# lis-epfl/multi_agent_pkgs

Measured on AMD Instinct MI355X. Metric: agent QP-replans/sec, higher is better.
Workload: dtype f64

## Files before the change

### __graft_entry__.py

```python
import os
import subprocess
import sys

ROOT = os.path.dirname(os.path.abspath(__file__))
if ROOT not in sys.path:
    sys.path.insert(0, ROOT)


def build() -> None:
    csrc = os.path.join(ROOT, "multi_agent_pkgs_amd", "csrc")
    subprocess.check_call(["make", "-C", csrc, "-s"])
    subprocess.check_call(["make", "-C", os.path.join(ROOT, "oracle"), "-s"])
    subprocess.check_call(["make", "-C", os.path.join(ROOT, "tests", "wave_emu"), "-s"])
    subprocess.check_call(["make", "-C", os.path.join(ROOT, "examples"), "-s"])
    subprocess.check_call(["make", "-C", os.path.join(ROOT, "ros"), "-s"])
    subprocess.check_call(["make", "-C", os.path.join(ROOT, "tests", "ros_shim"), "-s"])
    import multi_agent_pkgs_amd
    from multi_agent_pkgs_amd import lib
    L = lib.load()
    for name in lib.EXPORTS:
        getattr(L, name)
    print("build ok: libhdsm.so version 0x%x" % L.hdsm_version())


def smoke() -> None:
    import numpy as np
    sys.path.insert(0, os.path.join(ROOT, "tests"))
    import problems
    from multi_agent_pkgs_amd import lib
    from multi_agent_pkgs_amd.params import agile_params
    from oracle import pyoracle as orc

    prm = agile_params(10, max_rows_static=18)
    sn = problems.swarm_snapshot(prm, 16, seed=7, turn=True)
    args = [sn[k] for k in ("agent_id", "state", "ref", "n_poly", "n_rows", "A", "b", "plans", "has_plan")]
    sol = lib.Solver(prm, 16, 16, device=0)
    g = sol.replan(*args)
    o = orc.replan(prm, *args)
    assert (g["status"] == o["status"]).all(), (g["status"], o["status"])
    ok = o["status"] != 2
    dt = float(np.abs(g["traj"] - o["traj"])[ok].max())
    dj = float(np.abs(g["obj"] - o["obj"])[ok].max())
    assert dt < 1e-6 and dj < 1e-6, (dt, dj)
    print("smoke ok: 16 agent-replans on cuda:0, max |traj - oracle| = %.2e, |obj - oracle| = %.2e" % (dt, dj))


# ... 5 lines not shown
```

### multi_agent_pkgs_amd/csrc/hdsm_consts.cpp

```cpp
#include "hdsm_consts.h"

#include <cmath>
#include <cstdlib>
#include <cstring>
#include <vector>

namespace hdsm {
namespace {

struct M3 {
  double m[3][3];
};
M3 eye() {
  M3 r{};
  for (int i = 0; i < 3; ++i) r.m[i][i] = 1;
  return r;
}
M3 mul(const M3& a, const M3& b) {
  M3 r{};
  for (int i = 0; i < 3; ++i)
    for (int j = 0; j < 3; ++j)
      for (int k = 0; k < 3; ++k) r.m[i][j] += a.m[i][k] * b.m[k][j];
  return r;
}
// ... 38 lines not shown
      char* end = nullptr;
      const long v = std::strtol(e, &end, 10);
      if (end != e && *end == 0 && v >= lo && v <= hi) *out = (int32_t)v;
    }
  };
  auto env_real = [](const char* name, double lo, double hi, double* out) {
    if (const char* e = std::getenv(name)) {
      char* end = nullptr;
      const double v = std::strtod(e, &end);
      if (end != e && *end == 0 && v >= lo && v <= hi) *out = v;
    }
  };
  if (prm->presweep < 0 || prm->presweep > 2) return fail(err, "presweep must be 0 (automatic), 1 (never) or 2 (always)");
  if (prm->branch_rule < 0 || prm->branch_rule > 1) return fail(err, "branch_rule must be 0 (most infeasible) or 1 (first in time)");
  if (prm->stage_radius < 0 || prm->time_limit_s < 0) return fail(err, "stage_radius / time_limit_s must not be negative");
  if (!(prm->mip_gap >= 0) || prm->mip_gap >= 1) return fail(err, "mip_gap must be in [0, 1)");
  c->cand_tau = prm->stage_radius > 0 ? prm->stage_radius : 0.6;
  env_real("HDSM_CAND_TAU", 0.01, 10.0, &c->cand_tau);
  c->branch_rule = prm->branch_rule == 0 ? 1 : 0;
  env_int("HDSM_BRANCH_RULE", 0, 1, &c->branch_rule);
  c->presweep = prm->presweep == 0 ? 2 : (prm->presweep == 1 ? 0 : 1);
  env_int("HDSM_PRESWEEP", 0, 2, &c->presweep);
  c->hot_tau = 1e30;
  env_real("HDSM_HOT_TAU", 1e-3, 1e30, &c->hot_tau);
  c->pick_rule = 1;
  env_int("HDSM_PICK_RULE", 0, 1, &c->pick_rule);
  c->box_cut = 1;
  env_int("HDSM_BOX_CUT", 0, 1, &c->box_cut);
  c->scanner = 1;
  env_int("HDSM_SCANNER", 0, 2, &c->scanner);
  c->child_bound = 1, c->overlap_sweep = 1;
  env_int("HDSM_OVERLAP_SWEEP", 0, 1, &c->overlap_sweep);
  env_int("HDSM_CHILD_BOUND", 0, 1, &c->child_bound);
  c->dominance = 1;
  env_int("HDSM_DOMINANCE", 0, 1, &c->dominance);
  c->mip_gap = prm->mip_gap;
  c->leaf_mfma = 1;
  env_int("HDSM_LEAF_MFMA", 0, 1, &c->leaf_mfma);
  c->time_ticks = 0;
  c->r_u = prm->r_u;
  for (int k = 0; k < 6; ++k) c->wx[k] = prm->r_x[k], c->wn[k] = prm->r_n[k];
  for (int ax = 0; ax < 3; ++ax) {
    c->lbu[ax] = prm->u_lb[ax], c->ubu[ax] = prm->u_ub[ax];
    for (int comp = 1; comp < 3; ++comp) {
      c->lbs[comp][ax] = prm->x_lb[3 * comp + ax];
      c->ubs[comp][ax] = prm->x_ub[3 * comp + ax];
    }
  }
  c->radius = prm->drone_radius;
  const double kk = prm->drone_radius / prm->drone_z_offset;
  c->k2m1 = kk * kk - 1.0;
  c->pert = prm->plane_perturb;

  for (int ax = 0; ax < 3; ++ax) {
    M3 Ac{};
    Ac.m[0][1] = 1, Ac.m[1][1] = -prm->drag[ax], Ac.m[1][2] = 1;
    const double dt = prm->dt;
    M3 Ad, Bm;
    if (!prm->rk4) {
      Ad = axpy(eye(), dt, Ac);
      Bm = eye();
      for (auto& row : Bm.m)
        for (double& v : row) v *= dt;
    } else {
      const M3 A1 = Ac, A2 = mul(Ac, Ac), A3 = mul(A2, Ac), A4 = mul(A3, Ac);
      Ad = axpy(axpy(axpy(axpy(eye(), dt, A1), dt * dt / 2, A2), dt * dt * dt / 6, A3), dt * dt * dt * dt / 24, A4);
// ... 227 lines not shown
```

### multi_agent_pkgs_amd/csrc/hdsm_core.h

```cpp
#pragma once
#include <math.h>
#include <stdint.h>

#include <hip/hip_runtime.h>
#define HD __device__ __forceinline__
#define HDN __device__ __noinline__
#define PAR_FOR(i, cnt) for (int i = tid_here(); i < (cnt); i += (int)blockDim.x)
#define HDSM_UNROLL _Pragma("unroll")
#define SYNC() __syncthreads()
#define IS_T0 (HDSM_TX == 0)
namespace hdsm {
__device__ __forceinline__ int atomic_inc_i32(int* p) { return atomicAdd(p, 1); }
__device__ __forceinline__ unsigned tx() {
  unsigned t = threadIdx.x;
#if defined(__HIP_DEVICE_COMPILE__)
  asm volatile("" : "+v"(t));
#endif
  return t;
}
}
#define HDSM_TX (hdsm::tx())
#if defined(__HIP_DEVICE_COMPILE__)
#define HDSM_KERNARG_WORD __attribute__((address_space(4))) long long
#else
#define HDSM_KERNARG_WORD long long
#endif

#include "hdsm_types.h"

namespace hdsm {

enum { GI_OK = 0, GI_INFEASIBLE = 1, GI_CUTOFF = 2, GI_ITERLIM = 3, GI_DONE = 4, GI_TIMELIM = 5 };
constexpr int NODE_CHUNK = 4;
constexpr int TREE_MARK = 32;
constexpr int WARM_CERT = 1 << 30;
enum { FLAG_NODE_LIMIT = 1, FLAG_ITER_LIMIT = 2, FLAG_TIME_LIMIT = 4, FLAG_STAGING_OVERFLOW = 8 };
enum { ST_OPTIMAL = 0, ST_LIMIT = 1, ST_NO_SOLUTION = 2, ST_PENDING = 3 };

enum { K_U = 0, K_S = 1, K_P = 2, K_C = 3, K_E = 4 };
HD int mk_id(int kind, int payload) { return (kind << 28) | payload; }
HD int id_kind(int id) { return (id >> 28) & 7; }
HD int id_payload(int id) { return id & 0x0fffffff; }
HD int mk_kc(int slot, int m) { return mk_id(K_C, (m << 12) | slot); }
HD int kc_slot(int payload) { return payload & 0xfff; }
HD int kc_m(int payload) { return payload >> 12; }

constexpr int LISTCAP = 768;

struct alignas(8) MW {
  int32_t m;
  float w;
};
static_assert(sizeof(MW) == 8, "hand-over records copy MW as one 8-byte word");
HD MW mk_mw(const double (*kap)[4], double nx, double ny, double nz, int m) {
  const double q = nx * nx * kap[m][0] + ny * ny * kap[m][1] + nz * nz * kap[m][2];
  return MW{m, q > 1e-60 ? (float)(1.0 / sqrt(q)) : 1e30f};
}

template <int NV, int CMAX, bool SMALL = false>
struct Shm {
  static_assert(CMAX <= 4096, "the slot of a staged row must fit the 12 bits kc_slot() reads");
  static constexpr int PM = SMALL ? 4 : MAXP, RSM = SMALL ? 20 : MAXRS, LC = SMALL ? 512 : LISTCAP;
  static constexpr int LDT = (NV <= 32) ? 34 : NV + 2;
  alignas(16) double T[2];
  alignas(16) double U[NV * LDT];
  alignas(16) double dvec[NV + 2];
  alignas(16) double dvz[NV + 2];
  double gz[3][3][2 * MAXH];
  double x0[NV];
  double fx0;
  int32_t cand_src[CMAX];
  int32_t inc_act[NV], inc_nact;
  int32_t st_sph, st_pairs;
  long long t_start;
#ifdef HDSM_PROFILE
  long long prof_acc[24];
  long long prof_last;
  long long prof_last1;
#endif
  double x[NV], lam[NV], w[NV], grad[NV];
  double inc_x[NV];
  double g[3][3][MAXH];
  double fr[3][MAXH + 1][3];
  double ref[MAXH][6];
  double st[MAXH + 1][9];
  double cprev[MAXH][3];
  alignas(16) double sp[PM][RSM][4];
  double keys[MAXH][PM];
  static constexpr int HTS = NV / 3;
  double br_lb[HTS][PM], br_pv[HTS][PM];
  int32_t br_pk[HTS][PM];
  HD double& lb_at(int item) { return red_v[item]; }
  HD double& pv_at(int item) { return red_v[64 + item]; }
  HD int32_t& pk_at(int item) { return reinterpret_cast<int32_t*>(&red_v[128])[item]; }
  static_assert(128 + 32 <= MAXT, "the leaf test's per-(step, polyhedron) values fit the reduction scratch");
// ... 2 lines not shown
  double first_v;
  double lb_top1, lb_top2;
  int32_t lb_step;
  alignas(16) double cand[CMAX][4];
  double red_v[MAXT];
  double br_f[MAXH];
  double state0[9];
  double f, inc_f, f0;
  MW cand_mw[CMAX];
  int32_t act[NV];
  int32_t sp_rows[PM];
  int32_t assign[MAXH], contain[MAXH], inc_assign[MAXH];
  int32_t br_step[MAXH], br_pos[MAXH], br_cnt[MAXH], br_order[MAXH][PM];
  int32_t q, neq_done, ncand, n_poly, level, have_inc, fixed_bad, overflow;
  int32_t inf_id;
  unsigned long long nogood[NOGOODS];
  int32_t n_nogood, ng_skipped, ng_global;
  int32_t lb_skipped;
  int32_t ncold;
  double f_box;
  double inc_shared;
  int32_t wanted_raw;
  int32_t nviol;
  int32_t warm_head;
  int32_t warm_ncand;
  int32_t leaf_pick;
  int32_t sp_dom, dom_done;
  int32_t forced;
  double* snap;
  int32_t node_res;
  int32_t rc, iters_sh;
  int32_t cmd;
  int32_t nlist;
  int32_t grp[2];
  int32_t list[LC];
  double sw[5];
  double sw_ref[MAXH + 1][3];
  double sw_tau;
  double sw_d2;
  double bnd[24];
  static_assert(MAXT >= 16 + KCOLS + 8, "the reduction scratch doubles as the set-up's input vector");
  HD double* vin() { return &red_v[16]; }
  double part_v[4];
  double part_key[4];
  double part_tol;
  int32_t part_id[4];
  int32_t part_norm;
  double kap[MAXH + 1][4];
  Args args;
};

HD bool tasc_plane_eval(const Consts& c, const double* cp, const double* op, double* out) {
  const double dx = op[0] - cp[0], dy = op[1] - cp[1], dz = op[2] - cp[2];
  const double n2 = dx * dx + dy * dy + dz * dz;
  if (!(n2 > 0)) return false;
  const double nrm = sqrt(n2), inv = 1.0 / nrm;
  const double hx = dx * inv, hy = dy * inv, hz = dz * inv;
  const double sd = c.radius / sqrt(1.0 + c.k2m1 * hz * hz);
  const double back = 0.5 * fmin(2.0 * sd, nrm);
  const double qx = 0.5 * (cp[0] + op[0]) - back * hx;
  const double qy = 0.5 * (cp[1] + op[1]) - back * hy;
  const double qz = 0.5 * (cp[2] + op[2]) - back * hz;
  const double fx = hx + c.pert * (hy - hz) - c.pert * hz;
  const double fy = hy - c.pert * hx;
  const double fz = hz + c.pert * hx + c.pert * hx;
  out[0] = fx, out[1] = fy, out[2] = fz;
// ... 738 lines not shown
        s.f0 = t0;
        s.fx0 = t0 + 0.5 * t1;
        s.f = s.fx0 + 0.5 * t2;
        s.inc_nact = 0;
      }
    }
    SYNC();
    SU_PROF(15)

#ifdef HDSM_PROFILE
    const long long t_setup_ = clock64() - t_begin_;
#endif
#ifdef HDSM_TIMELINE
    const long long tl_setup_ = (long long)wall_clock64();
    long long tl_warm_ = 0, tl_sweep_ = 0, tl_run_ = 0, tl_leaf_ = 0;
    int tl_warm_it_ = 0, tl_runs_ = 0;
#define TL_T0 const long long tl_t0_ = (long long)wall_clock64();
#define TL_ADD(acc) acc += (long long)wall_clock64() - tl_t0_;
#else
#define TL_T0
#define TL_ADD(acc)
#endif
    int iters = 0, nodes = 1, sweeps = 0;
    bool warm_cert = false;
    if (a.warm != nullptr && np > 0) warm_cert = (s.warm_head & WARM_CERT) != 0;
#if defined(HDSM_PROFILE)
    long long t_warm_ = 0;
    int it_warm_ = 0;
#endif
    bool limit = false, handed_over = false;
    int rec_slot = -1;
    unsigned flags = 0;
    bool run = np > 0;
    if (IS_T0) s.sw_tau = 0.0;
    bool item_run = false;
    if (item >= 0) {
      const SplitRec& rc = a.recs[item >> 8];
      const int L = (item >> 3) & 15, pos = item & 7;
      const int nh = rc.ncand, ncl = rc.ncold;
      const int64_t rbase = (int64_t)(item >> 8) * a.rows_cap;
      SYNC();
      PAR_FOR(k, nh + ncl) {
        const int slot = k < nh ? k : CMAX - ncl + (k - nh);
        const double* src = a.rec_cand + (rbase + k) * 4;
        s.cand[slot][0] = src[0], s.cand[slot][1] = src[1], s.cand[slot][2] = src[2], s.cand[slot][3] = src[3];
        *reinterpret_cast<long long*>(&s.cand_mw[slot]) = a.rec_mw[rbase + k];
        s.cand_src[slot] = a.rec_src[rbase + k];
      }
      PAR_FOR(k, 3 * (N + 1)) s.sw_ref[k / 3][k % 3] = rc.sw_ref[k / 3][k % 3];
      PAR_FOR(k, rc.n_nogood) s.nogood[k] = rc.nogood[k];
      PAR_FOR(l, L + 1) {
        s.br_step[l] = rc.br_step[l], s.br_cnt[l] = 0, s.br_pos[l] = 0, s.br_f[l] = rc.br_f[l];
        s.assign[rc.br_step[l]] = l < L ? rc.assign[rc.br_step[l]] : rc.br_order[L][pos];
      }
      if (IS_T0) {
        s.ncand = nh, s.ncold = ncl, s.n_nogood = rc.n_nogood, s.sw_tau = rc.sw_tau, s.level = L + 1;
        s.sp_dom = rc.sp_dom, s.dom_done = 1;
        const int code = rc.br_pk[L][pos];
        s.first_id = code >= 0 ? mk_id(K_P, (rc.br_step[L] << 7) | code) : -1, s.first_v = rc.br_pv[L][pos];
        const unsigned long long bits = __hip_atomic_load(&a.inc_bits[inst], __ATOMIC_RELAXED, __HIP_MEMORY_SCOPE_AGENT);
        s.inc_shared = __longlong_as_double((long long)bits);
      }
      SYNC();
      item_run = run && nh + ncl <= CMAX && !(rc.br_lb[L][pos] >= cutoff(s, c));
      if (item_run) snapshot_io(s, c, R, const_cast<double*>(rc.snap) + (int64_t)L * SNAP_STRIDE, false);
      if (IS_T0) s.neq_done = 6;
      run = item_run;
// ... 537 lines not shown
```

### multi_agent_pkgs_amd/csrc/hdsm_types.h

```cpp
#pragma once
#include <stdint.h>

namespace hdsm {

constexpr int MAXH = 16;
constexpr int MAXP = 8;
constexpr int MAXRS = 32;
constexpr int MAXNV = 3 * MAXH;
constexpr int MAXT = 256;
constexpr int KCOLS = 9 + 6 * MAXH;
constexpr int KROWS = 3 * MAXNV + 12;
constexpr int SPLIT_N_MAX = 30;
constexpr int KCH = 3 + 2 * MAXH;
constexpr double ABSENT = 1e20;
constexpr double DINF = 1e300;

struct Consts {
  int32_t N, n, P, RS;
  int32_t max_nodes, max_iters;
  int32_t presweep;
  int32_t leaf_mfma;
  int32_t branch_rule;
  int32_t pick_rule;
  int32_t box_cut;
  int32_t scanner;
  int32_t child_bound;
  int32_t overlap_sweep;
  double tol, ftol_fixed, cand_tau, hot_tau;
  double mip_gap;
  long long time_ticks;
  double r_u, wx[6], wn[6];
  double lbu[3], ubu[3];
  double lbs[3][3], ubs[3][3];
  double radius, k2m1, pert;
  double Ad[3][3][3], Bd[3][3];
  double g[3][3][MAXH];
  int32_t pinned_steps;
  int32_t dominance;
  double phi[3][MAXH + 1][3][3];
  double Hinv[MAXNV * MAXNV];
  double J0[MAXNV * MAXNV];
  double Jeq[MAXNV * MAXNV];
  double Req[36], Ueq[36];
  double Meq[MAXNV * 6];
  double Seq[36];
  double KT[KCOLS * KROWS];
  double KTC[KCH * KROWS];
  int32_t kax[KROWS];
  double JeqP[MAXNV * 64];
  double hrow1[MAXNV];
  double wu[MAXNV];
  double ws[3][3][MAXH + 1];
  double kap[MAXH + 1][4];
};

constexpr int NOGOODS = 48;
constexpr int ITEMS_PER_REC = 64;

struct SplitRec {
  int32_t inst, level, ncand, ncold, n_nogood, first_item, n_items, nodes_done, sweeps_done, truncated;
// ... 77 lines not shown
```

### multi_agent_pkgs_amd/csrc/hdsm_wave_gi.h

```cpp
#pragma once
#include <hip/hip_runtime.h>

#include "hdsm_types.h"

namespace hdsm {

template <int CTRL>
__device__ __forceinline__ double dpp64(double v) {
  int lo = __double2loint(v), hi = __double2hiint(v);
  lo = __builtin_amdgcn_mov_dpp(lo, CTRL, 0xf, 0xf, true);
  hi = __builtin_amdgcn_mov_dpp(hi, CTRL, 0xf, 0xf, true);
  return __hiloint2double(hi, lo);
}
__device__ __forceinline__ double bcast64(double v, int lane) {
  const int lo = __builtin_amdgcn_readlane(__double2loint(v), lane);
  const int hi = __builtin_amdgcn_readlane(__double2hiint(v), lane);
  return __hiloint2double(hi, lo);
}
__device__ __forceinline__ double wave_max64(double v) {
  v = fmax(v, dpp64<0x121>(v));
  v = fmax(v, dpp64<0x122>(v));
  v = fmax(v, dpp64<0x124>(v));
  v = fmax(v, dpp64<0x128>(v));
  return fmax(fmax(bcast64(v, 0), bcast64(v, 16)), fmax(bcast64(v, 32), bcast64(v, 48)));
// ... 68 lines not shown
  if (hot) {
    slot = __hip_atomic_fetch_add(&ncand, 1, __ATOMIC_ACQ_REL, __HIP_MEMORY_SCOPE_WORKGROUP);
    const int other = __hip_atomic_load(&ncold, __ATOMIC_RELAXED, __HIP_MEMORY_SCOPE_WORKGROUP);
    return slot >= 0 && slot < CMAX - other;
  }
  slot = CMAX - 1 - __hip_atomic_fetch_add(&ncold, 1, __ATOMIC_ACQ_REL, __HIP_MEMORY_SCOPE_WORKGROUP);
  const int other = __hip_atomic_load(&ncand, __ATOMIC_RELAXED, __HIP_MEMORY_SCOPE_WORKGROUP);
  return slot < CMAX && slot >= other && slot >= 0;
#else
  slot = hot ? atomicAdd(&ncand, 1) : CMAX - 1 - atomicAdd(&ncold, 1);
  const bool fits = (hot ? slot < CMAX - __hip_atomic_load(&ncold, __ATOMIC_RELAXED, __HIP_MEMORY_SCOPE_WORKGROUP)
                         : slot >= __hip_atomic_load(&ncand, __ATOMIC_RELAXED, __HIP_MEMORY_SCOPE_WORKGROUP)) &&
                    slot >= 0 && slot < CMAX;
  HDSM_STAGE_AUDIT_CLAIM(slot, fits);
  return fits;
#endif
}

__device__ __forceinline__ void keep_in_loop(int& v) {
#if defined(__HIP_DEVICE_COMPILE__)
  asm volatile("" : "+v"(v));
#else
  (void)v;
#endif
}

__device__ __forceinline__ int tid_here() {
  int t = (int)HDSM_TX;
  keep_in_loop(t);
  return t;
}

__device__ __forceinline__ void keep_here(double& v) {
#if defined(__HIP_DEVICE_COMPILE__)
  asm volatile("" : "+v"(v));
#else
  (void)v;
#endif
}

template <class T>
__device__ __forceinline__ T* keep_in_loop(T* p) {
#if defined(__HIP_DEVICE_COMPILE__)
  asm volatile("" : "+v"(p));
#endif
  return p;
}

struct alignas(16) D2 {
  double x, y;
};

#if defined(__HIP_DEVICE_COMPILE__)
template <class T>
using GPtr = __attribute__((address_space(1))) T*;
template <class T>
__device__ __forceinline__ GPtr<const T> gptr(const T* p) { return (GPtr<const T>)p; }
template <class T>
__device__ __forceinline__ GPtr<T> gptr(T* p) { return (GPtr<T>)p; }
#else
template <class T>
using GPtr = T*;
template <class T>
__device__ __host__ inline GPtr<const T> gptr(const T* p) { return p; }
template <class T>
__device__ __host__ inline GPtr<T> gptr(T* p) { return p; }
// ... 87 lines not shown
        w.has = g.has_plan[k], w.ox = op[0], w.oy = op[1], w.oz = op[2];
      }
    }
  }

  struct LaneReq {
    double hrow;
    double wu, sb_w[2];
    int comp[2], axs[2], ii[2];
  };
  static __device__ __forceinline__ LaneReq init_lane_request(const Consts& c, int lane) {
    const int n = c.n;
    LaneReq q;
    q.wu = c.wu[lane < n ? lane : 0];
    q.hrow = c.hrow1[lane < n ? lane : 0];
#pragma unroll
    for (int e = 0; e < 2; ++e) {
      const int idx = lane + 64 * e, k = idx % 6;
      q.ii[e] = idx / 6 + 1, q.comp[e] = 1 + k / 3, q.axs[e] = k % 3;
      q.sb_w[e] = c.ws[q.axs[e]][q.comp[e]][q.ii[e] <= MAXH ? q.ii[e] : 0];
    }
    return q;
  }
  static __device__ __forceinline__ void init_lane(Regs& R, const Consts& c, int lane, const LaneReq& q) {
    const int N = c.N;
    const int n_sb = 6 * (N - 1);
    R.ax = row_of(lane) / N, R.kk = row_of(lane) % N;
    R.wu = (float)q.wu;
#pragma unroll
    for (int e = 0; e < 2; ++e) {
      const bool on = lane + 64 * e < n_sb;
      R.sb_id[e] = on ? ((q.ii[e] << 5) | (q.comp[e] << 3) | (q.axs[e] << 1)) : -1;
      R.sb_w[e] = (float)q.sb_w[e];
    }
  }

  template <int PART = 0>
  static __device__ __forceinline__ void states(S& s, const Regs& R, int lane, int N) {
    if constexpr (SPLIT) {
      constexpr bool P0 = PART != 2, VA = PART != 1;
      const int row = lane & 31, h = lane >> 5;
      const bool on = row < 3 * N;
      const int ax = on ? R.ax : 0, m = on ? R.kk + 1 : 1;
      double acc0 = 0, acc1 = 0, acc2 = 0;
      if (h == 0) {
        if constexpr (P0) acc0 = s.fr[ax][m][0];
        if constexpr (VA) acc1 = s.fr[ax][m][1], acc2 = s.fr[ax][m][2];
      }
      const double* xx = s.x + ax * N;
      const double* g0 = &s.gz[ax][0][MAXH + m - 1];
      const double* g1 = &s.gz[ax][1][MAXH + m - 1];
      const double* g2 = &s.gz[ax][2][MAXH + m - 1];
      constexpr int HH = HT / 2;
      static_assert(HT % 2 == 0, "the split kernel halves the horizon capacity");
#pragma unroll
      for (int k = 0; k < HH; ++k) {
        const int kk = h * HH + k;
        const double xk = xx[kk];
        if constexpr (P0) acc0 += g0[-kk] * xk;
        if constexpr (VA) acc1 += g1[-kk] * xk, acc2 += g2[-kk] * xk;
      }
      if constexpr (P0) acc0 = half_sum64(acc0);
      if constexpr (VA) acc1 = half_sum64(acc1), acc2 = half_sum64(acc2);
      if (on && h == 0) {
        if constexpr (P0) s.st[m][ax] = acc0;
        if constexpr (VA) s.st[m][3 + ax] = acc1, s.st[m][6 + ax] = acc2;
      }
// ... 250 lines not shown
  }

  template <bool SOLO = false>
  static __device__ __forceinline__ void sweep_planes(S& s, const Consts& c, const Args& a, int self, double thresh,
                                                      bool check_fixed, int lane, const double* pts = nullptr, int pstride = 9) {
    const int N = c.N, nt = SOLO ? 64 : (int)blockDim.x;
    if (pts == nullptr) pts = &s.st[0][0];
    const GPtr<const double> g_bounds = gptr(a.bounds), g_pos = gptr(a.pos);
    const GPtr<const uint8_t> g_has = gptr(a.has_plan);
    auto bar = [&]() {
      if constexpr (SOLO) wsync();
      else __syncthreads();
    };
    PROF_DECL
    const double radius = c.radius, k2m1 = c.k2m1, pert = c.pert, tol = c.tol, hot_tau = c.hot_tau;
    const int pinned = c.pinned_steps;
    const bool pre = a.bounds != nullptr;
    if (lane < 64) {
      double d2 = 0.0, r2 = 0.0;
      const double mx = 0.5 * (s.cprev[0][0] + s.cprev[N - 1][0]), my = 0.5 * (s.cprev[0][1] + s.cprev[N - 1][1]),
                   mz = 0.5 * (s.cprev[0][2] + s.cprev[N - 1][2]);
      if (lane < 2 * N) {
        const int i = lane >> 1, m = i + (lane & 1);
        const double* pm0 = pts + m * pstride;
        const double ux = pm0[0] - s.cprev[i][0], uy = pm0[1] - s.cprev[i][1], uz = pm0[2] - s.cprev[i][2];
        d2 = ux * ux + uy * uy + uz * uz;
        const double wx = s.cprev[i][0] - mx, wy = s.cprev[i][1] - my, wz = s.cprev[i][2] - mz;
        r2 = wx * wx + wy * wy + wz * wz;
      }
      d2 = wave_max64(d2), r2 = wave_max64(r2);
      if (lane == 0) {
        const double smax = radius * fmax(1.0, rsqrt_nr(1.0 + k2m1));
        const double nfmax = sqrt(1.0 + 9.0 * pert * pert);
        s.sw[0] = 2.0 * (fmax(thresh, tol) + smax + nfmax * sqrt(d2)) * (1.0 + 1e-9);
        s.sw[1] = mx, s.sw[2] = my, s.sw[3] = mz, s.sw[4] = sqrt(r2) * (1.0 + 1e-9);
        s.nlist = 0;
        HDSM_STAGE_AUDIT_BEGIN(s.ncand, s.ncold, CMAX);
      }
    }
    bar();
    const double cull = s.sw[0], cull2 = cull * cull;
    SW_PROF(8)
    const int g_lo = uni(s.grp[0]), g_hi = uni(s.grp[1]);
    const int chunk = pre ? S::LC : (g_hi > g_lo ? g_hi - g_lo : 1);
    for (int base = g_lo; base < g_hi; base += chunk) {
      const int end = (base + chunk < g_hi) ? base + chunk : g_hi;
      int cnt = end - base;
      if (pre) {
        const double sx = s.sw[1], sy = s.sw[2], sz = s.sw[3], reach0 = cull + s.sw[4];
        constexpr int FB = 4;
        for (int k0 = base + lane; k0 < end; k0 += FB * nt) {
          double4 bk[FB];
#pragma unroll
          for (int f = 0; f < FB; ++f) {
            const int k = k0 + f * nt;
            bk[f] = *(GPtr<const double4>)(g_bounds + 4 * (int64_t)(k < end ? k : base));
          }
#pragma unroll
          for (int f = 0; f < FB; ++f) {
            const int k = k0 + f * nt;
            const double ux = bk[f].x - sx, uy = bk[f].y - sy, uz = bk[f].z - sz, reach = reach0 + bk[f].w;
            if (k < end && k != self && bk[f].w >= 0 && !(ux * ux + uy * uy + uz * uz > reach * reach))
              s.list[atomicAdd(&s.nlist, 1)] = k;
          }
        }
        bar();
        cnt = s.nlist;
        SW_PROF(9)
      }
      const int total = cnt * N;
      if (lane == 0) s.st_sph += pre ? (end - base) : 0, s.st_pairs += total;
      for (int idx0 = 0; idx0 < total; idx0 += nt) {
        const int idx = idx0 + lane;
        const bool in = idx < total;
        const int j = in ? idx / N : 0, i = in ? idx - j * N : 0;
        const int k = in ? (pre ? s.list[j] : base + j) : 0;
        const GPtr<const double> op = g_pos + ((int64_t)k * N + i) * 3;
        const double ox = op[0], oy = op[1], oz = op[2];
        const bool on = in && k != self && (pre || g_has[k]);
        SW_PROF(10)
        const double cx = s.cprev[i][0], cy = s.cprev[i][1], cz = s.cprev[i][2];
        const double dx = ox - cx, dy = oy - cy, dz = oz - cz;
        const double n2 = dx * dx + dy * dy + dz * dz;
        if (on && n2 > 0 && n2 < cull2) {
          const double inv = rsqrt_nr(n2), nrm = n2 * inv;
          const double hx = dx * inv, hy = dy * inv, hz = dz * inv;
          const double sd = radius * rsqrt_nr(1.0 + k2m1 * hz * hz);
          const double back = 0.5 * fmin(2.0 * sd, nrm);
          const double qx = 0.5 * (cx + ox) - back * hx, qy = 0.5 * (cy + oy) - back * hy,
                       qz = 0.5 * (cz + oz) - back * hz;
          const double fx = hx + pert * (hy - hz) - pert * hz, fy = hy - pert * hx, fz = hz + 2.0 * pert * hx;
          const double rhs = fx * qx + fy * qy + fz * qz;
#pragma unroll
          for (int e = 0; e < 2; ++e) {
            const int m = i + e;
            const double* pm = pts + m * pstride;
            const double v = fx * pm[0] + fy * pm[1] + fz * pm[2] - rhs;
            if (m <= pinned) {
              if (check_fixed && v > c.ftol_fixed) s.fixed_bad = 1;
              continue;
            }
            if (v > tol) s.nviol = 1;
            if (-v < thresh) {
              const bool hot = -v < hot_tau;
              int slot;
              const bool fits = stage_slot<CMAX>(s.ncand, s.ncold, hot, slot);
              if (fits) {
                s.cand[slot][0] = fx, s.cand[slot][1] = fy, s.cand[slot][2] = fz, s.cand[slot][3] = rhs;
                s.cand_mw[slot] = mk_mw(s.kap, fx, fy, fz, m);
                s.cand_src[slot] = (k << 6) | (i << 1) | e;
              } else {
                s.overflow = 1;
// ... 30 lines not shown
```

### multi_agent_pkgs_amd/csrc/hdsm_wave_gib.h

```cpp
#pragma once
#include "hdsm_wave_gi.h"

namespace hdsm {

__device__ __forceinline__ double row16_sum64(double v) {
  const int lo = __double2loint(v), hi = __double2hiint(v);
  const auto a = __builtin_amdgcn_permlane16_swap(lo, lo, false, false);
  const auto b = __builtin_amdgcn_permlane16_swap(hi, hi, false, false);
  return __hiloint2double(b[0], a[0]) + __hiloint2double(b[1], a[1]);
}

struct Pair64 {
  double v, s;
};
__device__ __forceinline__ Pair64 swap16(double a, double b) {
  const auto lo = __builtin_amdgcn_permlane16_swap(__double2loint(a), __double2loint(b), false, false);
  const auto hi = __builtin_amdgcn_permlane16_swap(__double2hiint(a), __double2hiint(b), false, false);
  return Pair64{__hiloint2double(hi[0], lo[0]), __hiloint2double(hi[1], lo[1])};
}
__device__ __forceinline__ Pair64 swap32(double a, double b) {
  const auto lo = __builtin_amdgcn_permlane32_swap(__double2loint(a), __double2loint(b), false, false);
  const auto hi = __builtin_amdgcn_permlane32_swap(__double2hiint(a), __double2hiint(b), false, false);
  return Pair64{__hiloint2double(hi[0], lo[0]), __hiloint2double(hi[1], lo[1])};
}

template <int NVT, int CMAX, bool SMALL = false>
struct WaveGIB : WaveGI<NVT, CMAX, SMALL> {
  using Base = WaveGI<NVT, CMAX, SMALL>;
  using S = typename Base::S;
  using Regs = typename Base::Regs;
  static constexpr bool SPLIT = Base::SPLIT;
  static constexpr int NV = NVT, NC = Base::NC, NB = NC / 16, LDT = S::LDT;
  static_assert(NVT == 32 || NVT == 48, "two layouts");

// ... 42 lines not shown
  static __device__ __forceinline__ void gather_cols(double v, double (&g)[NC]) {
    if constexpr (SPLIT) {
      g[0] = v;
      gather_block(g);
    } else {
      const Pair64 a = swap16(v, v);
      const Pair64 b = swap32(a.v, a.v);
      const Pair64 c = swap32(a.s, a.s);
      g[0] = b.v, g[16] = c.v, g[32] = b.s;
#pragma unroll
      for (int bb = 0; bb < NB; ++bb) gather_block(g + 16 * bb);
    }
  }
  static __device__ __forceinline__ double pos_sum(double v, int lane) { return wave_sum64(first_copy(lane) ? v : 0.0); }

  static __device__ __forceinline__ void load_pos(const S& s, Regs& R, int lane) {
    R.lam = s.lam[pos_addr(lane)], R.act = first_copy(lane) || SPLIT ? s.act[pos_addr(lane)] : -1;
  }
  static __device__ __forceinline__ void store_pos(S& s, const Regs& R, int lane) {
    if (first_copy(lane)) s.lam[pos_of(lane)] = R.lam, s.act[pos_of(lane)] = R.act;
  }

  static __device__ __forceinline__ double u_row_dot(const S& s, int lane) {
    const int k = pos_addr(lane), c0 = ucol0(lane);
    const D2* urow = reinterpret_cast<const D2*>(&s.U[k * LDT + c0]);
    const D2* dv = reinterpret_cast<const D2*>(&s.dvec[c0]);
    double r0 = 0, r1 = 0;
#pragma unroll
    for (int j = 0; j < NC / 2; ++j) {
      const D2 u = urow[j], d = dv[j];
      r0 += u.x * d.x, r1 += u.y * d.y;
    }
    return psum(r0 + r1);
  }

  static constexpr int CMD_PICK = 2, CMD_PREP = 3;
  struct Refl {
    double rho, inv_rho, beta;
  };
  static __device__ __forceinline__ Refl reflection(double zz, double dq) {
    const double zs = zz > 0 ? zz : 1.0;
    const double inv_rho_abs = rsq_nr(zs);
    Refl h;
    h.rho = (dq > 0 ? -1.0 : 1.0) * (zs * inv_rho_abs), h.inv_rho = (dq > 0 ? -1.0 : 1.0) * inv_rho_abs;
    h.beta = rcp_nr(h.rho * (h.rho - dq));
    return h;
  }

  template <bool WANT_Z = true, bool WANT_DD = true>
  static __device__ __forceinline__ void direction(S& s, const Regs& R, double ai, int q, int lane, double& dj, double& dz,
                                                   double& dd, double& zz, double& dq, double& zi, double& ri, int prep_msg = 0,
                                                   Refl* refl = nullptr) {
    double p[NC];
    const double na = -ai;
#pragma unroll
    for (int k = 0; k < NC; ++k) p[k] = R.Jr[k] * na;
    dj = reduce_cols(p, lane);
    if constexpr (WANT_Z) { OP_PROF(12) }
    const int pos = pos_of(lane);
    if (first_copy(lane)) s.dvec[pos] = dj;
    dz = (pos >= q) ? dj : 0.0;
    dd = WANT_DD ? pos_sum(dj * dj, lane) : 0.0;
    zz = pos_sum(dz * dz, lane);
    dq = (q < NV) ? bcast64(dj, lane_of_pos(q < NV ? q : 0)) : 0.0;
    zi = 0.0;
    if (refl != nullptr) *refl = reflection(zz, dq);
// ... 75 lines not shown
      for (int j = 0; j < NC; j += 2) {
        const D2 v2 = ro[j / 2];
        ur[j] = v2.x, ur[j + 1] = v2.y;
      }
    }
    const double urt = s.U[pa * LDT + t];
    double wu0 = 0, wu1 = 0;
#pragma unroll
    for (int j = 0; j < NC; j += 2) wu0 += ur[j] * uv[j], wu1 += ur[j + 1] * uv[j + 1];
    const double cu = (psum(wu0 + wu1) - sigma * urt) * beta;
#pragma unroll
    for (int j = 0; j < NC; ++j) ur[j] -= cu * uv[j];
    if (first_copy(lane)) s.lam[pos] = R.lam, s.act[pos] = R.act;
    wsync();
    if (pos != l && pos < q) {
      D2* dst = reinterpret_cast<D2*>(&s.U[(pos > l ? pos - 1 : pos) * LDT + c0]);
#pragma unroll
      for (int j = 0; j < NC; j += 2) dst[j / 2] = D2{ur[j], ur[j + 1]};
    }
    if (pos >= l && pos < t) R.lam = s.lam[pos + 1], R.act = s.act[pos + 1];
    if (pos == t) R.lam = 0.0, R.act = -1;
    wsync();
    if (first_copy(lane)) s.U[pos * LDT + t] = 0.0;
    if (pos == t) {
      D2* dst = reinterpret_cast<D2*>(&s.U[pos * LDT + c0]);
#pragma unroll
      for (int j = 0; j < NC; j += 2) dst[j / 2] = D2{0.0, 0.0};
    }
    wsync();
  }

  using WarmPre = typename Base::WarmPre;
  using Base::warm_prefetch;
  static __device__ __forceinline__ void warm_start(S& s, const Consts& c, const Args& a, Regs& R, int inst, int self, int& iters,
                                                    const WarmPre& wpre, bool conc = false) {
    const int lane = (int)HDSM_TX;
    const int N = c.N, n = c.n;
    int nw = uni(wpre.head) & ~WARM_CERT;
    if (nw <= 0) {
      if (conc) {
        if (lane == 0) s.warm_ncand = s.ncand;
        __syncthreads();
      }
      return;
    }
    if (nw > NV) nw = NV;
    PROF_DECL
    int pre = -1, my_m = 0, my_src = 0;
    double my_row[4] = {0.0, 0.0, 0.0, 0.0};
    if (lane < nw) {
      const int code = wpre.code;
      const int kind = id_kind(code), p = id_payload(code);
      if (kind == K_U) {
        const int var = p >> 1;
        if (var % N >= 1) pre = mk_id(K_U, ((var - 1) << 1) | (p & 1));
      } else if (kind == K_S) {
        const int i = p >> 5;
        if (i - 1 >= 1) pre = mk_id(K_S, ((i - 1) << 5) | (p & 31));
      } else if (kind == K_C && a.l1_rows == nullptr) {
        const int e = p & 1, i = ((p >> 1) & 31) - 1, k = p >> 6;
        if (i >= 0 && i + e > c.pinned_steps && k != self && k >= s.grp[0] && k < s.grp[1] && wpre.has) {
          const double op[3] = {wpre.ox, wpre.oy, wpre.oz};
          if (tasc_plane_eval(c, s.cprev[i], op, my_row)) pre = -2, my_m = i + e, my_src = (k << 6) | (i << 1) | e;
        }
      }
    }
    int q = uni(s.q);
    const int q_in = q;
    load_pos(s, R, lane);
    {
      const unsigned long long want = __ballot(pre == -2);
      if (want != 0ull) {
        const int base = uni(s.ncand), room = CMAX - uni(s.ncold) - base;
        const int rank = __popcll(want & ((1ull << lane) - 1ull));
        if (pre == -2) {
          if (rank < room) {
            const int slot = base + rank;
            s.cand[slot][0] = my_row[0], s.cand[slot][1] = my_row[1], s.cand[slot][2] = my_row[2], s.cand[slot][3] = my_row[3];
            s.cand_mw[slot] = mk_mw(s.kap, my_row[0], my_row[1], my_row[2], my_m);
            s.cand_src[slot] = my_src;
            pre = mk_kc(slot, my_m);
          } else {
            pre = -1;
          }
        }
        const int cnt = __popcll(want);
        if (lane == 0) s.ncand = base + (cnt < room ? cnt : (room > 0 ? room : 0));
        wsync();
      }
    }
    if (conc) {
      if (lane == 0) s.warm_ncand = s.ncand;
      __syncthreads();
    }
    WS_PROF(16)
    for (int g = 0; g < nw && q < n; ++g) {
      const int id = __builtin_amdgcn_readlane(pre, g);
      if (id < 0) continue;
      WS_PROF(17)
      double ai;
      if (id_kind(id) == K_C) {
        const double nx = bcast64(my_row[0], g), ny = bcast64(my_row[1], g), nz = bcast64(my_row[2], g);
        const int m = kc_m(id_payload(id)), var = Base::row_of(lane);
        const double nax = R.ax == 0 ? nx : (R.ax == 1 ? ny : nz);
        ai = (var < n && R.kk < m) ? nax * s.gz[R.ax][0][MAXH + m - 1 - R.kk] : 0.0;
      } else {
        ai = Base::normal_entry(s, R, id, Base::row_of(lane), N, n);
      }
      WS_PROF(18)
      double dj, dz, dd, zz, dq, zi, ri;
      direction<false>(s, R, ai, q, lane, dj, dz, dd, zz, dq, zi, ri);
      WS_PROF(19)
      ++iters;
      if (!(zz > 1e-8 * dd)) continue;
      householder_add(s, R, id, 0.0, q, lane, dz, zz, dq, ri);
      WS_PROF(20)
      ++q;
    }
    if (q == q_in) return;
    if (lane < NV) s.x[lane] = s.x0[lane];
    store_pos(s, R, lane);
    wsync();
    Base::states(s, R, lane, N);
    const int pos = pos_of(lane), pa = pos_addr(lane), c0 = ucol0(lane);
    for (;;) {
      const double vk = (pos < q) ? Base::resid(s, c, R.act, N) : 0.0;
      if (first_copy(lane)) s.dvec[pos] = vk;
      wsync();
      double tj;
      {
        double p0 = 0, p1 = 0;
#pragma unroll
        for (int k = 0; k < NC; k += 2) {
          const D2 vk2 = *reinterpret_cast<const D2*>(&s.dvec[c0 + k]);
          p0 += s.U[(c0 + k) * LDT + pa] * vk2.x, p1 += s.U[(c0 + k + 1) * LDT + pa] * vk2.y;
        }
        tj = psum(p0 + p1);
      }
      wsync();
      if (first_copy(lane)) s.dvec[pos] = tj;
      wsync();
      const double lk = u_row_dot(s, lane);
      const bool ineq = pos < q && id_kind(R.act) != K_E;
      const double worst = -wave_max64(ineq ? -lk : -DINF);
      if (!(worst < -1e-12) || q <= 6) {
        double xw;
        {
          double g[NC];
          gather_cols(tj, g);
          double x0 = 0, x1 = 0;
#pragma unroll
          for (int k = 0; k < NC; k += 2) x0 += R.Jr[k] * g[k], x1 += R.Jr[k + 1] * g[k + 1];
          xw = s.x0[row_addr(lane)] + Base::hsum(x0 + x1);
        }
        const double tt = pos_sum(tj * tj, lane);
        R.lam = (pos < q) ? lk : 0.0;
        if (lane < n) R.xi = xw, s.x[lane] = xw;
        else if (lane < 64 && Base::row_ok(lane) && Base::row_of(lane) < n) R.xi = xw;
        if (lane == 0) s.f = s.fx0 + 0.5 * tt, s.q = q;
        store_pos(s, R, lane);
        wsync();
        WS_PROF(21)
        return;
      }
      const int l = pos_of(uni(__ffsll((long long)__ballot(ineq && lk == worst)) - 1));
      WS_PROF(21)
      drop(s, R, l, q, lane);
      WS_PROF(22)
      --q;
      ++iters;
    }
  }

  static __device__ __forceinline__ int run(S& s, const Consts& c, Regs& R, double f_cut, int& iters) {
    const int lane = (int)HDSM_TX;
    const int n = c.n, N = c.N, max_iters = c.max_iters;
    const double tol = c.tol;
    const long long time_ticks = c.time_ticks;
    const bool norm_pick = c.pick_rule != 0;
    double f = s.f;
    int q = uni(s.q), neq = uni(s.neq_done);
    int rc = GI_OK;
    const int pos = pos_of(lane);
    load_pos(s, R, lane);
    const bool duo = blockDim.x > 64 && c.scanner != 0;
    bool pending = false;
    int first_id = uni(s.first_id);
    if (lane == 0) s.first_id = -1;
    PROF_DECL
    for (;;) {
      int ln = lane;
      keep_in_loop(ln);
      int ip;
      double vip, kip = 0.0;
      double ai;
      if (neq < 6) {
        Base::states(s, R, ln, N);
        PROF(0)
        ip = mk_id(K_E, neq);
// ... 407 lines not shown
```

Baseline: 9.842 million.

## Cache and reuse the sphere-culled neighbour list across sweeps with gap-quantized entries

The neighbour pre-cull now runs as a single pass when the candidates fit in the shared list. Each entry packs a quantized clearance gap next to the agent id. On later sweeps over the same group range with a cull radius no larger than before, the cached list is filtered by that gap instead of re-reading all bounding spheres from global memory. The bound loads and the per-pair position loads are also software-prefetched one or two iterations ahead. This adds register pressure and extra barriers, falls back to chunked sweeping when the list overflows, and relies on the quantized gap being conservative to stay correct.

```diff
diff --git a/__graft_entry__.py b/__graft_entry__.py
--- a/__graft_entry__.py
+++ b/__graft_entry__.py
@@ -12,6 +12,7 @@
     subprocess.check_call(["make", "-C", csrc, "-s"])
     subprocess.check_call(["make", "-C", os.path.join(ROOT, "oracle"), "-s"])
     subprocess.check_call(["make", "-C", os.path.join(ROOT, "tests", "wave_emu"), "-s"])
+    subprocess.check_call(["make", "-C", os.path.join(ROOT, "tests", "sweep_emu"), "-s"])
     subprocess.check_call(["make", "-C", os.path.join(ROOT, "examples"), "-s"])
     subprocess.check_call(["make", "-C", os.path.join(ROOT, "ros"), "-s"])
     subprocess.check_call(["make", "-C", os.path.join(ROOT, "tests", "ros_shim"), "-s"])
diff --git a/multi_agent_pkgs_amd/csrc/hdsm_consts.cpp b/multi_agent_pkgs_amd/csrc/hdsm_consts.cpp
--- a/multi_agent_pkgs_amd/csrc/hdsm_consts.cpp
+++ b/multi_agent_pkgs_amd/csrc/hdsm_consts.cpp
@@ -94,6 +94,8 @@
   c->child_bound = 1, c->overlap_sweep = 1;
   env_int("HDSM_OVERLAP_SWEEP", 0, 1, &c->overlap_sweep);
   env_int("HDSM_CHILD_BOUND", 0, 1, &c->child_bound);
+  c->sweep_list = 1;
+  env_int("HDSM_SWEEP_LIST", 0, 1, &c->sweep_list);
   c->dominance = 1;
   env_int("HDSM_DOMINANCE", 0, 1, &c->dominance);
   c->mip_gap = prm->mip_gap;
diff --git a/multi_agent_pkgs_amd/csrc/hdsm_core.h b/multi_agent_pkgs_amd/csrc/hdsm_core.h
--- a/multi_agent_pkgs_amd/csrc/hdsm_core.h
+++ b/multi_agent_pkgs_amd/csrc/hdsm_core.h
@@ -45,7 +45,15 @@
 HD int kc_slot(int payload) { return payload & 0xfff; }
 HD int kc_m(int payload) { return payload >> 12; }
 
-constexpr int LISTCAP = 768;
+#ifdef HDSM_TEST_LISTCAP
+constexpr int LISTCAP = HDSM_TEST_LISTCAP, LISTCAP_SMALL = HDSM_TEST_LISTCAP;
+#else
+constexpr int LISTCAP = 768, LISTCAP_SMALL = 512;
+#endif
+enum { SW_CHUNKS = 0, SW_PASS = 1, SW_REUSE = 2 };
+constexpr int SW_IDS = 1 << 16;
+constexpr double SW_GAP_SCALE = 1024.0;
+constexpr int SW_REUSE_MIN = 256;
 
 struct alignas(8) MW {
   int32_t m;
@@ -60,7 +68,7 @@
 template <int NV, int CMAX, bool SMALL = false>
 struct Shm {
   static_assert(CMAX <= 4096, "the slot of a staged row must fit the 12 bits kc_slot() reads");
-  static constexpr int PM = SMALL ? 4 : MAXP, RSM = SMALL ? 20 : MAXRS, LC = SMALL ? 512 : LISTCAP;
+  static constexpr int PM = SMALL ? 4 : MAXP, RSM = SMALL ? 20 : MAXRS, LC = SMALL ? LISTCAP_SMALL : LISTCAP;
   static constexpr int LDT = (NV <= 32) ? 34 : NV + 2;
   alignas(16) double T[2];
   alignas(16) double U[NV * LDT];
@@ -129,6 +137,8 @@
   int32_t rc, iters_sh;
   int32_t cmd;
   int32_t nlist;
+  int32_t list_ok, sw_mode, list_rng[2];
+  double list_cull;
   int32_t grp[2];
   int32_t list[LC];
   double sw[5];
@@ -933,7 +943,7 @@
     int rec_slot = -1;
     unsigned flags = 0;
     bool run = np > 0;
-    if (IS_T0) s.sw_tau = 0.0;
+    if (IS_T0) s.sw_tau = 0.0, s.list_ok = 0;
     bool item_run = false;
     if (item >= 0) {
       const SplitRec& rc = a.recs[item >> 8];
diff --git a/multi_agent_pkgs_amd/csrc/hdsm_types.h b/multi_agent_pkgs_amd/csrc/hdsm_types.h
--- a/multi_agent_pkgs_amd/csrc/hdsm_types.h
+++ b/multi_agent_pkgs_amd/csrc/hdsm_types.h
@@ -26,6 +26,7 @@
   int32_t scanner;
   int32_t child_bound;
   int32_t overlap_sweep;
+  int32_t sweep_list;
   double tol, ftol_fixed, cand_tau, hot_tau;
   double mip_gap;
   long long time_ticks;
diff --git a/multi_agent_pkgs_amd/csrc/hdsm_wave_gi.h b/multi_agent_pkgs_amd/csrc/hdsm_wave_gi.h
--- a/multi_agent_pkgs_amd/csrc/hdsm_wave_gi.h
+++ b/multi_agent_pkgs_amd/csrc/hdsm_wave_gi.h
@@ -594,9 +594,14 @@
       if (lane == 0) {
         const double smax = radius * fmax(1.0, rsqrt_nr(1.0 + k2m1));
         const double nfmax = sqrt(1.0 + 9.0 * pert * pert);
-        s.sw[0] = 2.0 * (fmax(thresh, tol) + smax + nfmax * sqrt(d2)) * (1.0 + 1e-9);
+        const double cull_now = 2.0 * (fmax(thresh, tol) + smax + nfmax * sqrt(d2)) * (1.0 + 1e-9);
+        s.sw[0] = cull_now;
         s.sw[1] = mx, s.sw[2] = my, s.sw[3] = mz, s.sw[4] = sqrt(r2) * (1.0 + 1e-9);
-        s.nlist = 0;
+        int mode = SW_CHUNKS;
+        if (pre && c.sweep_list != 0)
+          mode = (s.list_ok != 0 && cull_now <= s.list_cull && s.list_rng[0] == s.grp[0] && s.list_rng[1] == s.grp[1]) ? SW_REUSE : SW_PASS;
+        s.sw_mode = mode;
+        if (mode != SW_REUSE) s.nlist = 0, s.list_ok = 0;
         HDSM_STAGE_AUDIT_BEGIN(s.ncand, s.ncold, CMAX);
       }
     }
@@ -604,42 +609,114 @@
     const double cull = s.sw[0], cull2 = cull * cull;
     SW_PROF(8)
     const int g_lo = uni(s.grp[0]), g_hi = uni(s.grp[1]);
-    const int chunk = pre ? S::LC : (g_hi > g_lo ? g_hi - g_lo : 1);
+    int mode = pre ? uni(s.sw_mode) : SW_CHUNKS;
+    const bool packed = a.n_rob <= SW_IDS;
+    const int idmask = packed ? SW_IDS - 1 : -1;
+    if (mode == SW_REUSE) {
+      const int n0 = uni(s.nlist), qmax = (int)fmin(cull * SW_GAP_SCALE, 65535.0) + 1;
+      bar();
+      if (lane == 0) s.nlist = 0;
+      bar();
+      for (int r0 = 0; r0 < n0; r0 += nt) {
+        const bool in = r0 + lane < n0;
+        const uint32_t e = in ? (uint32_t)s.list[r0 + lane] : 0u;
+        bar();
+        if (in && (int)(e >> 16) <= qmax) s.list[atomicAdd(&s.nlist, 1)] = (int32_t)e;
+        bar();
+      }
+      if (lane == 0) s.list_cull = cull;
+      SW_PROF(9)
+    }
+    int chunk = (pre && mode == SW_CHUNKS) ? S::LC : (g_hi > g_lo ? g_hi - g_lo : 1);
     for (int base = g_lo; base < g_hi; base += chunk) {
       const int end = (base + chunk < g_hi) ? base + chunk : g_hi;
       int cnt = end - base;
-      if (pre) {
-        const double sx = s.sw[1], sy = s.sw[2], sz = s.sw[3], reach0 = cull + s.sw[4];
+      if (pre && mode != SW_REUSE) {
+        const double sx = s.sw[1], sy = s.sw[2], sz = s.sw[3], reach0 = cull + s.sw[4], rho = s.sw[4];
+        const bool gaps = packed && mode == SW_PASS;
         constexpr int FB = 4;
-        for (int k0 = base + lane; k0 < end; k0 += FB * nt) {
-          double4 bk[FB];
+        double4 bk[FB], nx[FB];
+#pragma unroll
+        for (int f = 0; f < FB; ++f) {
+          const int k = base + lane + f * nt;
+          bk[f] = *(GPtr<const double4>)(g_bounds + 4 * (int64_t)(k < end ? k : base));
+        }
+        for (int k0 = base; k0 < end; k0 += FB * nt) {
+          const bool more = k0 + FB * nt < end;
+          if (more) {
+#pragma unroll
+            for (int f = 0; f < FB; ++f) {
+              const int k = k0 + FB * nt + lane + f * nt;
+              nx[f] = *(GPtr<const double4>)(g_bounds + 4 * (int64_t)(k < end ? k : base));
+            }
+          }
 #pragma unroll
           for (int f = 0; f < FB; ++f) {
-            const int k = k0 + f * nt;
-            bk[f] = *(GPtr<const double4>)(g_bounds + 4 * (int64_t)(k < end ? k : base));
+            const int k = k0 + lane + f * nt;
+            const double ux = bk[f].x - sx, uy = bk[f].y - sy, uz = bk[f].z - sz, reach = reach0 + bk[f].w;
+            const double u2 = ux * ux + uy * uy + uz * uz;
+            if (k < end && k != self && bk[f].w >= 0 && !(u2 > reach * reach)) {
+              int q = 0;
+              if (gaps && bk[f].w < 1e299) {
+                const double gap = sqrt(u2) - bk[f].w - rho;
+                if (gap > 0) q = (int)fmin(gap * SW_GAP_SCALE, 65535.0);
+                q = q > 0 ? q - 1 : 0;
+              }
+              const int slot = atomicAdd(&s.nlist, 1);
+              if (slot < S::LC) s.list[slot] = packed ? (int32_t)(((uint32_t)q << 16) | (uint32_t)k) : k;
+            }
           }
-#pragma unroll
-          for (int f = 0; f < FB; ++f) {
-            const int k = k0 + f * nt;
-            const double ux = bk[f].x - sx, uy = bk[f].y - sy, uz = bk[f].z - sz, reach = reach0 + bk[f].w;
-            if (k < end && k != self && bk[f].w >= 0 && !(ux * ux + uy * uy + uz * uz > reach * reach))
-              s.list[atomicAdd(&s.nlist, 1)] = k;
+          if (more) {
+#pragma unroll
+            for (int f = 0; f < FB; ++f) bk[f] = nx[f];
           }
         }
         bar();
         cnt = s.nlist;
+        if (lane == 0) s.st_sph += end - base;
         SW_PROF(9)
+        if (mode == SW_PASS) {
+          if (cnt > S::LC) {
+            bar();
+            if (lane == 0) s.nlist = 0;
+            bar();
+            mode = SW_CHUNKS, chunk = S::LC, base = g_lo - chunk;
+            continue;
+          }
+          if (lane == 0) s.list_ok = (packed && g_hi - g_lo >= SW_REUSE_MIN) ? 1 : 0, s.list_cull = cull, s.list_rng[0] = g_lo, s.list_rng[1] = g_hi;
+        }
+      } else if (pre) {
+        cnt = uni(s.nlist);
       }
       const int total = cnt * N;
-      if (lane == 0) s.st_sph += pre ? (end - base) : 0, s.st_pairs += total;
-      for (int idx0 = 0; idx0 < total; idx0 += nt) {
-        const int idx = idx0 + lane;
+      if (lane == 0) s.st_pairs += total;
+      struct PairReq {
+        double ox, oy, oz;
+        int k, i;
+        bool on;
+      };
+      auto request = [&](int idx) {
         const bool in = idx < total;
         const int j = in ? idx / N : 0, i = in ? idx - j * N : 0;
-        const int k = in ? (pre ? s.list[j] : base + j) : 0;
+        const int k = in ? (pre ? (s.list[j] & idmask) : base + j) : 0;
         const GPtr<const double> op = g_pos + ((int64_t)k * N + i) * 3;
-        const double ox = op[0], oy = op[1], oz = op[2];
-        const bool on = in && k != self && (pre || g_has[k]);
+        PairReq r;
+        r.ox = op[0], r.oy = op[1], r.oz = op[2];
+        r.k = k, r.i = i, r.on = in && k != self && (pre || g_has[k]);
+        return r;
+      };
+      constexpr int PD = 2;
+      PairReq rq[PD];
+#pragma unroll
+      for (int d = 0; d < PD; ++d) rq[d] = request(d * nt < total ? d * nt + lane : total);
+      for (int idx0 = 0; idx0 < total; idx0 += nt) {
+        const PairReq p = rq[0];
+#pragma unroll
+        for (int d = 0; d + 1 < PD; ++d) rq[d] = rq[d + 1];
+        if (idx0 + PD * nt < total) rq[PD - 1] = request(idx0 + PD * nt + lane);
+        const int k = p.k, i = p.i;
+        const double ox = p.ox, oy = p.oy, oz = p.oz;
+        const bool on = p.on;
         SW_PROF(10)
         const double cx = s.cprev[i][0], cy = s.cprev[i][1], cz = s.cprev[i][2];
         const double dx = ox - cx, dy = oy - cy, dz = oz - cz;
```

New measurement: 9.760 million, median of 2. About the same (-0.8%).

## Screen warm-start candidates by incremental multiplier sign before Householder install

Applied to the files above, without the earlier changes.

In the SPLIT variant, warm start now computes the transformed residual vector once up front and updates it incrementally as each candidate constraint is added. Inequality candidates whose new multiplier would be negative are rejected before the Householder update, which avoids adding rows that would later be dropped, and the first U^T·v recomputation is skipped. The non-split path keeps the old behaviour in a factored-out install_plain routine. Register pinning hints on sb_w, sb_id and wu were also added for SPLIT. The change adds audit hooks and relies on an extended householder_add signature, and rejecting candidates early may alter which active set the solver ends up with.

```diff
diff --git a/multi_agent_pkgs_amd/csrc/hdsm_wave_gi.h b/multi_agent_pkgs_amd/csrc/hdsm_wave_gi.h
--- a/multi_agent_pkgs_amd/csrc/hdsm_wave_gi.h
+++ b/multi_agent_pkgs_amd/csrc/hdsm_wave_gi.h
@@ -124,6 +124,14 @@
 }
 
 __device__ __forceinline__ void keep_here(double& v) {
+#if defined(__HIP_DEVICE_COMPILE__)
+  asm volatile("" : "+v"(v));
+#else
+  (void)v;
+#endif
+}
+
+__device__ __forceinline__ void keep_here(float& v) {
 #if defined(__HIP_DEVICE_COMPILE__)
   asm volatile("" : "+v"(v));
 #else
@@ -277,7 +285,9 @@
       const bool on = lane + 64 * e < n_sb;
       R.sb_id[e] = on ? ((q.ii[e] << 5) | (q.comp[e] << 3) | (q.axs[e] << 1)) : -1;
       R.sb_w[e] = (float)q.sb_w[e];
-    }
+      if constexpr (SPLIT) keep_here(R.sb_w[e]), keep_in_loop(R.sb_id[e]);
+    }
+    if constexpr (SPLIT) keep_here(R.wu);
   }
 
   template <int PART = 0>
diff --git a/multi_agent_pkgs_amd/csrc/hdsm_wave_gib.h b/multi_agent_pkgs_amd/csrc/hdsm_wave_gib.h
--- a/multi_agent_pkgs_amd/csrc/hdsm_wave_gib.h
+++ b/multi_agent_pkgs_amd/csrc/hdsm_wave_gib.h
@@ -1,5 +1,12 @@
 #pragma once
 #include "hdsm_wave_gi.h"
+
+#ifndef HDSM_WARM_AUDIT
+#define HDSM_WARM_AUDIT(event)
+#endif
+namespace hdsm {
+enum WarmEvent { WARM_EV_REJECT = 0, WARM_EV_ACCEPT, WARM_EV_DROP_NEW, WARM_EV_DROP_OLD, WARM_EV_BOX_ROW, WARM_EV_COUNT };
+}
 
 namespace hdsm {
 
@@ -108,6 +115,21 @@
       r0 += u.x * d.x, r1 += u.y * d.y;
     }
     return psum(r0 + r1);
+  }
+
+  static __device__ __forceinline__ double ut_dot(S& s, double vk, int lane) {
+    const int pos = pos_of(lane), pa = pos_addr(lane), c0 = ucol0(lane);
+    if (first_copy(lane)) s.dvec[pos] = vk;
+    wsync();
+    double p0 = 0, p1 = 0;
+#pragma unroll
+    for (int k = 0; k < NC; k += 2) {
+      const D2 vk2 = *reinterpret_cast<const D2*>(&s.dvec[c0 + k]);
+      p0 += s.U[(c0 + k) * LDT + pa] * vk2.x, p1 += s.U[(c0 + k + 1) * LDT + pa] * vk2.y;
+    }
+    const double tj = psum(p0 + p1);
+    wsync();
+    return tj;
   }
 
   static constexpr int CMD_PICK = 2, CMD_PREP = 3;
@@ -249,6 +271,89 @@
 
   using WarmPre = typename Base::WarmPre;
   using Base::warm_prefetch;
+  static constexpr bool WARM_PROBE = SPLIT;
+  static __device__ __forceinline__ void install_plain(S& s, const Consts& c, Regs& R, int lane, int nw, int pre, const double (&my_row)[4],
+                                                       int q, int& iters) {
+    const int N = c.N, n = c.n, q_in = q;
+    PROF_DECL
+    for (int g = 0; g < nw && q < n; ++g) {
+      const int id = __builtin_amdgcn_readlane(pre, g);
+      if (id < 0) continue;
+      WS_PROF(17)
+      double ai;
+      if (id_kind(id) == K_C) {
+        const double nx = bcast64(my_row[0], g), ny = bcast64(my_row[1], g), nz = bcast64(my_row[2], g);
+        const int m = kc_m(id_payload(id)), var = Base::row_of(lane);
+        const double nax = R.ax == 0 ? nx : (R.ax == 1 ? ny : nz);
+        ai = (var < n && R.kk < m) ? nax * s.gz[R.ax][0][MAXH + m - 1 - R.kk] : 0.0;
+      } else {
+        ai = Base::normal_entry(s, R, id, Base::row_of(lane), N, n);
+      }
+      WS_PROF(18)
+      double dj, dz, dd, zz, dq, zi, ri;
+      direction<false>(s, R, ai, q, lane, dj, dz, dd, zz, dq, zi, ri);
+      WS_PROF(19)
+      ++iters;
+      if (!(zz > 1e-8 * dd)) continue;
+      householder_add(s, R, id, 0.0, q, lane, dz, zz, dq, ri);
+      WS_PROF(20)
+      ++q;
+    }
+    if (q == q_in) return;
+    if (lane < NV) s.x[lane] = s.x0[lane];
+    store_pos(s, R, lane);
+    wsync();
+    Base::states(s, R, lane, N);
+    const int pos = pos_of(lane), pa = pos_addr(lane), c0 = ucol0(lane);
+    for (;;) {
+      const double vk = (pos < q) ? Base::resid(s, c, R.act, N) : 0.0;
+      if (first_copy(lane)) s.dvec[pos] = vk;
+      wsync();
+      double tj;
+      {
+        double p0 = 0, p1 = 0;
+#pragma unroll
+        for (int k = 0; k < NC; k += 2) {
+          const D2 vk2 = *reinterpret_cast<const D2*>(&s.dvec[c0 + k]);
+          p0 += s.U[(c0 + k) * LDT + pa] * vk2.x, p1 += s.U[(c0 + k + 1) * LDT + pa] * vk2.y;
+        }
+        tj = psum(p0 + p1);
+      }
+      wsync();
+      if (first_copy(lane)) s.dvec[pos] = tj;
+      wsync();
+      const double lk = u_row_dot(s, lane);
+      const bool ineq = pos < q && id_kind(R.act) != K_E;
+      const double worst = -wave_max64(ineq ? -lk : -DINF);
+      if (!(worst < -1e-12) || q <= 6) {
+        double xw;
+        {
+          double g[NC];
+          gather_cols(tj, g);
+          double x0 = 0, x1 = 0;
+#pragma unroll
+          for (int k = 0; k < NC; k += 2) x0 += R.Jr[k] * g[k], x1 += R.Jr[k + 1] * g[k + 1];
+          xw = s.x0[row_addr(lane)] + Base::hsum(x0 + x1);
+        }
+        const double tt = pos_sum(tj * tj, lane);
+        R.lam = (pos < q) ? lk : 0.0;
+        if (lane < n) R.xi = xw, s.x[lane] = xw;
+        else if (lane < 64 && Base::row_ok(lane) && Base::row_of(lane) < n) R.xi = xw;
+        if (lane == 0) s.f = s.fx0 + 0.5 * tt, s.q = q;
+        store_pos(s, R, lane);
+        wsync();
+        WS_PROF(21)
+        return;
+      }
+      const int l = pos_of(uni(__ffsll((long long)__ballot(ineq && lk == worst)) - 1));
+      WS_PROF(21)
+      drop(s, R, l, q, lane);
+      WS_PROF(22)
+      --q;
+      ++iters;
+    }
+  }
+
   static __device__ __forceinline__ void warm_start(S& s, const Consts& c, const Args& a, Regs& R, int inst, int self, int& iters,
                                                     const WarmPre& wpre, bool conc = false) {
     const int lane = (int)HDSM_TX;
@@ -311,10 +416,22 @@
       __syncthreads();
     }
     WS_PROF(16)
+    if constexpr (!WARM_PROBE) {
+      install_plain(s, c, R, lane, nw, pre, my_row, q, iters);
+      return;
+    }
+    const int pos = pos_of(lane);
+    if (lane < NV) s.x[lane] = s.x0[lane];
+    wsync();
+    Base::states(s, R, lane, N);
+    if (pre >= 0) s.w[lane] = Base::resid(s, c, pre, N);
+    if (pre >= 0 && id_kind(pre) != K_C) { HDSM_WARM_AUDIT(WARM_EV_BOX_ROW) }
+    double tj = ut_dot(s, (pos < q) ? Base::resid(s, c, R.act, N) : 0.0, lane);
     for (int g = 0; g < nw && q < n; ++g) {
       const int id = __builtin_amdgcn_readlane(pre, g);
       if (id < 0) continue;
       WS_PROF(17)
+      const double vg = s.w[g];
       double ai;
       if (id_kind(id) == K_C) {
         const double nx = bcast64(my_row[0], g), ny = bcast64(my_row[1], g), nz = bcast64(my_row[2], g);
@@ -329,32 +446,38 @@
       direction<false>(s, R, ai, q, lane, dj, dz, dd, zz, dq, zi, ri);
       WS_PROF(19)
       ++iters;
-      if (!(zz > 1e-8 * dd)) continue;
-      householder_add(s, R, id, 0.0, q, lane, dz, zz, dq, ri);
+      const double num = vg - pos_sum(pos < q ? dj * tj : 0.0, lane);
+      if (!(zz > 1e-8 * dd) || (id_kind(id) != K_E && num < -1e-12 * zz)) {
+        if (zz > 1e-8 * dd) { HDSM_WARM_AUDIT(WARM_EV_REJECT) }
+        continue;
+      }
+      const Refl refl = reflection(zz, dq);
+      const double tq = num * refl.inv_rho;
+      householder_add(s, R, id, 0.0, q, lane, dz, zz, dq, ri, &refl);
+      if (pos == q) tj = tq;
       WS_PROF(20)
       ++q;
-    }
-    if (q == q_in) return;
-    if (lane < NV) s.x[lane] = s.x0[lane];
+      HDSM_WARM_AUDIT(WARM_EV_ACCEPT)
+#ifdef HDSM_WARM_AUDIT_CHECK
+      {
+        const double tf = ut_dot(s, (pos < q) ? Base::resid(s, c, R.act, N) : 0.0, lane);
+        if (first_copy(lane)) s.dvec[pos] = tf;
+        wsync();
+        const double lf = u_row_dot(s, lane);
+        if (lane == lane_of_pos(q - 1)) { HDSM_WARM_AUDIT_CHECK(tq * refl.inv_rho, lf) }
+        wsync();
+      }
+#endif
+    }
+    if (q == q_in) {
+      if (lane < NV) s.x[lane] = R.xi;
+      wsync();
+      return;
+    }
     store_pos(s, R, lane);
     wsync();
-    Base::states(s, R, lane, N);
-    const int pos = pos_of(lane), pa = pos_addr(lane), c0 = ucol0(lane);
-    for (;;) {
-      const double vk = (pos < q) ? Base::resid(s, c, R.act, N) : 0.0;
-      if (first_copy(lane)) s.dvec[pos] = vk;
-      wsync();
-      double tj;
-      {
-        double p0 = 0, p1 = 0;
-#pragma unroll
-        for (int k = 0; k < NC; k += 2) {
-          const D2 vk2 = *reinterpret_cast<const D2*>(&s.dvec[c0 + k]);
-          p0 += s.U[(c0 + k) * LDT + pa] * vk2.x, p1 += s.U[(c0 + k + 1) * LDT + pa] * vk2.y;
-        }
-        tj = psum(p0 + p1);
-      }
-      wsync();
+    for (bool first = true;; first = false) {
+      if (!first) tj = ut_dot(s, (pos < q) ? Base::resid(s, c, R.act, N) : 0.0, lane);
       if (first_copy(lane)) s.dvec[pos] = tj;
       wsync();
       const double lk = u_row_dot(s, lane);
@@ -382,6 +505,7 @@
       }
       const int l = pos_of(uni(__ffsll((long long)__ballot(ineq && lk == worst)) - 1));
       WS_PROF(21)
+      HDSM_WARM_AUDIT(l >= q_in ? WARM_EV_DROP_NEW : WARM_EV_DROP_OLD)
       drop(s, R, l, q, lane);
       WS_PROF(22)
       --q;
```

Result: faster. 9.845 million before, 10.23 million after, median of 6 (+3.9%).
